# mokemokechicken/reversi-alpha-zero

Hardware: AMD Instinct MI355X
Metric: MCTS simulations/sec (self-play, NN included) (higher is better)
Workload: dtype f64 tree statistics + f32 net (f16x3 split-operand MFMA trunk)

## Files before the change

reversi-alpha-zero_amd/csrc/raz_net_f16x3.hip:

```cpp
#include <hip/hip_runtime.h>
#include <math.h>
#include <stdlib.h>
#include <string.h>
#include <vector>
#include "raz_bitboard.h"
#include "raz_detmath.h"
#include "raz_internal.h"
#include "raz_net_layout.h"

namespace {

typedef _Float16 h8 __attribute__((ext_vector_type(8)));
typedef _Float16 h4 __attribute__((ext_vector_type(4)));
typedef float f32x4 __attribute__((ext_vector_type(4)));
typedef float f32x16 __attribute__((ext_vector_type(16)));

constexpr int OCT = 128;
constexpr int NWAVE = 8;
constexpr int W_STAGE = 3 * 2 * 2 * OCT * 16;
constexpr int ACT_POS = 4 * 64 * 16;
constexpr int ACT_IMG = NWAVE * ACT_POS + 1280;
constexpr int LDS_W = 0;
constexpr int LDS_ACT = 2 * W_STAGE;
constexpr int LDS_BYTES = LDS_ACT + 2 * ACT_IMG;
constexpr int Z_OFF = NWAVE * ACT_POS;

#ifdef RAZ_F16X3_STAMPS
#define RAZ_STAMP_PARAM , unsigned long long* __restrict__ stamps
#define RAZ_STAMP_ARG , (unsigned long long*)nullptr
#define RAZ_STAMP_BEGIN                                                                                           \
    unsigned long long st_t[8];                                                                                   \
    st_t[0] = __builtin_amdgcn_s_memtime();                                                                       \
    st_t[7] = __builtin_amdgcn_s_memrealtime();                                                                   \
    st_t[6] = (unsigned long long)__builtin_amdgcn_s_getreg((4 << 0) | (0 << 6) | (31 << 11)) | ((unsigned long long)__builtin_amdgcn_s_getreg((20 << 0) | (0 << 6) | (31 << 11)) << 32); \
    st_t[5] = 0;                                                                                                  \
    st_t[1] = st_t[2] = st_t[3] = st_t[4] = 0;                                                                    \
    unsigned long long st_b = 0
#define RAZ_STAMP_BARRIER_IN st_b = __builtin_amdgcn_s_memtime()
#define RAZ_STAMP_BARRIER_OUT(st_)                                    \
    do {                                                              \
        const unsigned long long t_ = __builtin_amdgcn_s_memtime();   \
        st_t[5] += t_ - st_b;                                         \
        if ((st_) == 0) st_t[1] = t_;                                 \
    } while (0)
#define RAZ_STAMP_AT(i_) st_t[i_] = __builtin_amdgcn_s_memtime()
#define RAZ_STAMP_END                                                                                    \
    do {                                                                                                 \
        st_t[3] = __builtin_amdgcn_s_memtime();                                                          \
        __builtin_amdgcn_s_waitcnt(0x0070);                                                \
        st_t[4] = __builtin_amdgcn_s_memtime();                                                          \
        if (lane == 0 && stamps)                                                                         \
            for (int i_ = 0; i_ < 8; ++i_) stamps[((size_t)blockIdx.x * NWAVE + wv) * 8 + i_] = st_t[i_]; \
    } while (0)
#else
#define RAZ_STAMP_PARAM
#define RAZ_STAMP_ARG
#define RAZ_STAMP_BEGIN
#define RAZ_STAMP_BARRIER_IN
#define RAZ_STAMP_BARRIER_OUT(st_)
#define RAZ_STAMP_AT(i_)
#define RAZ_STAMP_END
#endif

__device__ __forceinline__ void halves_trade(float a, float b, int upper, float& first, float& second) {
#ifdef RAZ_WAVE_EMU
    const float got = __shfl_xor(upper ? a : b, 32);
    first = upper ? got : a;
    second = upper ? b : got;
#else
    (void)upper;
    const auto r = __builtin_amdgcn_permlane32_swap(__float_as_uint(a), __float_as_uint(b), false, false);
    first = __uint_as_float(r[0]);
    second = __uint_as_float(r[1]);
#endif
}

#define GLDS16(gptr, lptr)                                                                                      \
    __builtin_amdgcn_global_load_lds((const __attribute__((address_space(1))) void*)(gptr),                     \
                                     (__attribute__((address_space(3))) void*)(lptr), 16, 0, 0)

template <bool SPLIT>
__global__ __launch_bounds__(512, 2) void k_conv3x3_f16x3(const unsigned char* __restrict__ Wl, const float* __restrict__ bias,
                                                          const float* __restrict__ inv_scale_ptr, const unsigned char* in, unsigned char* out,
                                                          const unsigned char* skip, const uint8_t* __restrict__ active, int n, int F,
                                                          unsigned* __restrict__ flag, const uint32_t* __restrict__ n_ptr RAZ_STAMP_PARAM) {
    extern __shared__ __attribute__((aligned(16))) unsigned char lds[];
    const int tid = threadIdx.x, lane = tid & 63, wv = tid >> 6;
    RAZ_STAMP_BEGIN;
    if (n_ptr) n = (int)*n_ptr < n ? (int)*n_ptr : n;
    const int noct = F / OCT, nchunks = F / 16;
    const int b = blockIdx.x;
    const int ot = (b >> 3) % noct;
    const int pg = (b / (8 * noct)) * 8 + (b & 7);
    const int p0 = pg * NWAVE, pos = p0 + wv;
    if (p0 >= n) return;
    const bool live = pos < n && (!active || active[pos]);
    const size_t pos_bytes = (size_t)F * 256;
    const unsigned char* in_pos = in + (size_t)(pos < n ? pos : n - 1) * pos_bytes;
    if (tid < 160) {
        const int im = tid / 80, k = tid % 80;
        ((f32x4*)(lds + LDS_ACT + im * ACT_IMG + Z_OFF))[k] = (f32x4){0.f, 0.f, 0.f, 0.f};
    }
    const int kg = lane >> 5;
    uint32_t boff[2][9];
#pragma unroll
    for (int nt = 0; nt < 2; ++nt) {
        const int sq = nt * 32 + (lane & 31), y = sq >> 3, x = sq & 7;
#pragma unroll
        for (int t = 0; t < 9; ++t) {
            const int yy = y + t / 3 - 1, xx = x + t % 3 - 1;
            const bool ok = yy >= 0 && yy < 8 && xx >= 0 && xx < 8;
            const int s2 = sq + (t / 3 - 1) * 8 + (t % 3 - 1);
            boff[nt][t] = ok ? (uint32_t)(wv * ACT_POS + kg * 2048 + s2 * 16) : (uint32_t)(Z_OFF + (s2 & 15) * 16);
        }
    }
    const uint32_t aoff = (uint32_t)(kg * 4096 + (lane & 31) * 16);
    f32x16 acc[4][2];
#pragma unroll
    for (int m = 0; m < 4; ++m)
#pragma unroll
        for (int nt = 0; nt < 2; ++nt)
#pragma unroll
            for (int r = 0; r < 16; ++r) acc[m][nt][r] = 0.f;
    const unsigned char* wsrc = Wl + (size_t)ot * nchunks * 3 * W_STAGE + lane * 16;
    const unsigned char* asrc = in_pos + lane * 16;
    auto issue = [&](int c, int tg) {
        const int st = c * 3 + tg;
        const unsigned char* src = wsrc + (size_t)st * W_STAGE;
        unsigned char* dst = lds + LDS_W + (st & 1) * W_STAGE;
        if constexpr (SPLIT) {
#pragma unroll
            for (int i = 0; i < 3; ++i) GLDS16(src + (wv * 3 + i) * 1024, dst + (wv * 3 + i) * 1024);
        } else {
            const int p0w = (wv >> 1) * 4 + (wv & 1);
            GLDS16(src + p0w * 1024, dst + p0w * 1024);
            if (wv < 4) GLDS16(src + (p0w + 16) * 1024, dst + (p0w + 16) * 1024);
        }
        if (tg == 0) {
            const unsigned char* a = asrc + (size_t)c * ACT_POS;
            unsigned char* ad = lds + LDS_ACT + (c & 1) * ACT_IMG + wv * ACT_POS;
#pragma unroll
            for (int pl = 0; pl < 4; pl += SPLIT ? 1 : 2) GLDS16(a + pl * 1024, ad + pl * 1024);
        }
    };
    issue(0, 0);
    for (int c = 0; c < nchunks; ++c) {
        const uint32_t abase = (uint32_t)(LDS_ACT + (c & 1) * ACT_IMG);
#pragma unroll
        for (int tg = 0; tg < 3; ++tg) {
            const int st = c * 3 + tg;
            RAZ_STAMP_BARRIER_IN;
            __syncthreads();
            RAZ_STAMP_BARRIER_OUT(st);
            if (tg < 2) issue(c, tg + 1);
            else if (c + 1 < nchunks) issue(c + 1, 0);
            const uint32_t wbase = (uint32_t)(LDS_W + (st & 1) * W_STAGE) + aoff;
#pragma unroll
            for (int tt = 0; tt < 3; ++tt) {
                const int t = tg * 3 + tt;
                if constexpr (SPLIT) {
                    h8 bh[2], bl[2];
#pragma unroll
                    for (int nt = 0; nt < 2; ++nt) {
                        bh[nt] = *(const h8*)(lds + abase + boff[nt][t]);
                        bl[nt] = *(const h8*)(lds + abase + boff[nt][t] + 1024);
                    }
#pragma unroll
                    for (int m = 0; m < 4; ++m) {
                        const h8 ah = *(const h8*)(lds + wbase + tt * 8192 + m * 512);
                        const h8 al = *(const h8*)(lds + wbase + tt * 8192 + m * 512 + 2048);
#pragma unroll
                        for (int nt = 0; nt < 2; ++nt) {
                            acc[m][nt] = __builtin_amdgcn_mfma_f32_32x32x16_f16(al, bh[nt], acc[m][nt], 0, 0, 0);
                            acc[m][nt] = __builtin_amdgcn_mfma_f32_32x32x16_f16(ah, bl[nt], acc[m][nt], 0, 0, 0);
                            acc[m][nt] = __builtin_amdgcn_mfma_f32_32x32x16_f16(ah, bh[nt], acc[m][nt], 0, 0, 0);
                        }
                    }
                } else {
                    h8 bh[2];
#pragma unroll
                    for (int nt = 0; nt < 2; ++nt) bh[nt] = *(const h8*)(lds + abase + boff[nt][t]);
#pragma unroll
                    for (int m = 0; m < 4; ++m) {
                        const h8 ah = *(const h8*)(lds + wbase + tt * 8192 + m * 512);
#pragma unroll
                        for (int nt = 0; nt < 2; ++nt) acc[m][nt] = __builtin_amdgcn_mfma_f32_32x32x16_f16(ah, bh[nt], acc[m][nt], 0, 0, 0);
                    }
                }
            }
        }
    }
    RAZ_STAMP_AT(2);
    if (!live) return;
    const float inv_scale = *inv_scale_ptr;
    unsigned char* out_pos = out + (size_t)pos * pos_bytes + lane * 16;
    const unsigned char* skip_pos = skip ? skip + (size_t)pos * pos_bytes + lane * 16 : nullptr;
    h8 skh[2][4], skl[2][4];
    auto load_skip = [&](int m) {
#pragma unroll
        for (int q = 0; q < 4; ++q) {
            const int oc8 = ot * OCT + m * 32 + q * 8;
            const size_t unit = (size_t)(oc8 >> 4) * ACT_POS + (size_t)((oc8 >> 3) & 1) * 2048;
            skh[m & 1][q] = *(const h8*)(skip_pos + unit);
            if constexpr (SPLIT) skl[m & 1][q] = *(const h8*)(skip_pos + unit + 1024);
        }
    };
    if (skip_pos) load_skip(0);
    bool over = false;
#pragma unroll
    for (int m = 0; m < 4; ++m) {
        if (skip_pos && m + 1 < 4) load_skip(m + 1);
#pragma unroll
        for (int q = 0; q < 4; ++q) {
            const int oc8 = ot * OCT + m * 32 + q * 8;
            const size_t unit = (size_t)(oc8 >> 4) * ACT_POS + (size_t)((oc8 >> 3) & 1) * 2048;
            float v[8];
#pragma unroll
            for (int j = 0; j < 4; ++j) halves_trade(acc[m][0][q * 4 + j], acc[m][1][q * 4 + j], kg, v[j], v[4 + j]);
#pragma unroll
            for (int j = 0; j < 8; ++j) v[j] = v[j] * inv_scale + bias[oc8 + j];
            if (skip_pos) {
                const h8 sh = skh[m & 1][q];
                if constexpr (SPLIT) {
                    const h8 sl = skl[m & 1][q];
#pragma unroll
                    for (int j = 0; j < 8; ++j) v[j] = v[j] + ((float)sh[j] + (float)sl[j]);
                } else {
#pragma unroll
                    for (int j = 0; j < 8; ++j) v[j] = v[j] + (float)sh[j];
                }
            }
            h8 hi, lo;
#pragma unroll
            for (int j = 0; j < 8; ++j) {
                const float r = v[j] > 0.0f ? v[j] : 0.0f;
                over |= !(r < 60000.0f);
                hi[j] = (_Float16)r;
                lo[j] = (_Float16)(r - (float)hi[j]);
            }
            *(h8*)(out_pos + unit) = hi;
            if constexpr (SPLIT) *(h8*)(out_pos + unit + 1024) = lo;
        }
    }
    if (over) flag[(size_t)pos * RAZ_NET_ROWFLAG_WORDS] = 1u;
    RAZ_STAMP_END;
}

typedef float f32x2 __attribute__((ext_vector_type(2)));
constexpr int CONV0_ROWS = 2;

template <bool SPLIT>
__global__ __launch_bounds__(256, 6) void k_conv0_split(const float* __restrict__ W0, const raz_bb* __restrict__ own,
                                                        const raz_bb* __restrict__ enemy, const uint8_t* __restrict__ active,
                                                        unsigned char* out, int n, int F, unsigned* __restrict__ flag,
                                                        const uint32_t* __restrict__ list, const uint32_t* __restrict__ n_ptr) {
    const int posA = blockIdx.x * CONV0_ROWS, posB = posA + 1, lane = threadIdx.x & 63;
    const int wv = __builtin_amdgcn_readfirstlane(threadIdx.x >> 6);
    if (threadIdx.x == 0) {
        flag[(size_t)posA * RAZ_NET_ROWFLAG_WORDS] = 0u;
        if (posB < n) flag[(size_t)posB * RAZ_NET_ROWFLAG_WORDS] = 0u;
        if (posA == 0) flag[1] = 0u;
    }
    __syncthreads();
    if (n_ptr) n = (int)*n_ptr < n ? (int)*n_ptr : n;
    const bool liveA = posA < n && (list || !active || active[posA]);
    const bool liveB = posB < n && (list || !active || active[posB]);
    if (!liveA && !liveB) return;
    raz_bb bo[2] = {0, 0}, be[2] = {0, 0};
    if (liveA) {
        const size_t src = list ? list[posA] : (size_t)posA;
        bo[0] = own[src];
        be[0] = enemy[src];
    }
    if (liveB) {
        const size_t src = list ? list[posB] : (size_t)posB;
        bo[1] = own[src];
        be[1] = enemy[src];
    }
    const int y = lane >> 3, x = lane & 7;
    f32x2 x0[9], x1[9];
#pragma unroll
    for (int t = 0; t < 9; ++t) {
        const int yy = y + t / 3 - 1, xx = x + t % 3 - 1;
        const bool ok = (yy >= 0) && (yy < 8) && (xx >= 0) && (xx < 8);
        const int s = (yy * 8 + xx) & 63;
#pragma unroll
        for (int k = 0; k < 2; ++k) {
            x0[t][k] = ok ? (float)(uint32_t)((bo[k] >> s) & 1) : 0.0f;
            x1[t][k] = ok ? (float)(uint32_t)((be[k] >> s) & 1) : 0.0f;
        }
    }
    const float* bias = W0 + (size_t)F * 18;
    unsigned char* op = out + (size_t)posA * F * 256 + lane * 16;
    bool overA = false, overB = false;
    for (int ocb = wv; ocb < F / 16; ocb += 4) {
#pragma unroll 1
        for (int g = 0; g < 2; ++g) {
            f32x2 acc[8];
#pragma unroll
            for (int o = 0; o < 8; ++o) {
                const float b = bias[ocb * 16 + g * 8 + o];
                acc[o] = (f32x2){b, b};
            }
#pragma unroll
            for (int t = 0; t < 9; ++t) {
                const float* wt = W0 + ((size_t)ocb * 9 + t) * 32 + g * 8;
#pragma unroll
                for (int o = 0; o < 8; ++o) {
                    const float w = wt[o];
                    acc[o] = __builtin_elementwise_fma(x0[t], (f32x2){w, w}, acc[o]);
                }
#pragma unroll
                for (int o = 0; o < 8; ++o) {
                    const float w = wt[16 + o];
                    acc[o] = __builtin_elementwise_fma(x1[t], (f32x2){w, w}, acc[o]);
                }
            }
#pragma unroll
            for (int k = 0; k < 2; ++k) {
                if (!(k ? liveB : liveA)) continue;
                h8 hi, lo;
                bool over = false;
#pragma unroll
                for (int j = 0; j < 8; ++j) {
                    const float r = acc[j][k] > 0.0f ? acc[j][k] : 0.0f;
                    over |= !(r < 60000.0f);
                    hi[j] = (_Float16)r;
                    lo[j] = (_Float16)(r - (float)hi[j]);
                }
                if (k) overB |= over;
                else overA |= over;
                unsigned char* o16 = op + (size_t)k * F * 256 + (size_t)ocb * ACT_POS + (g * 2) * 1024;
                *(h8*)o16 = hi;
                if constexpr (SPLIT) *(h8*)(o16 + 1024) = lo;
            }
        }
    }
    if (overA) flag[(size_t)posA * RAZ_NET_ROWFLAG_WORDS] = 1u;
    if (overB) flag[(size_t)posB * RAZ_NET_ROWFLAG_WORDS] = 1u;
}

template <bool SPLIT>
__global__ __launch_bounds__(64) void k_heads_split(const float* __restrict__ H, const unsigned char* trunk,
                                                    const uint8_t* __restrict__ active, float* __restrict__ policy,
                                                    float* __restrict__ value, int n, int F, int V,
                                                    const uint32_t* __restrict__ list, const uint32_t* __restrict__ n_ptr) {
    extern __shared__ __attribute__((aligned(16))) float head[];
    const int pos = blockIdx.x, lane = threadIdx.x;
    if (n_ptr) n = (int)*n_ptr < n ? (int)*n_ptr : n;
    if (pos >= n || (!list && active && !active[pos])) return;
    const size_t dst = list ? list[pos] : (size_t)pos;
    const float* pol_w = H;
    const float* pol_b = pol_w + 2 * F;
    const float* pfc_w = pol_b + 2;
    const float* pfc_b = pfc_w + 128 * 64;
    const float* val_w = pfc_b + 64;
    const float* val_b = val_w + F;
    const float* v1_w = val_b + 1;
    const float* v1_b = v1_w + 64 * V;
    const float* v2_w = v1_b + V;
    const float* v2_b = v2_w + V;
    float* ph = head;
    float* vh = head + 128;
    float* h1 = head + 192;
    const unsigned char* a = trunk + (size_t)pos * F * 256 + lane * 16;
    float p0 = pol_b[0], p1 = pol_b[1], v0 = val_b[0];
    for (int c = 0; c < F / 16; ++c) {
#pragma unroll
        for (int g = 0; g < 2; ++g) {
            const h8 hi = *(const h8*)(a + (size_t)c * ACT_POS + (g * 2 + 0) * 1024);
            h8 lo = hi;
            if constexpr (SPLIT) lo = *(const h8*)(a + (size_t)c * ACT_POS + (g * 2 + 1) * 1024);
#pragma unroll
            for (int j = 0; j < 8; ++j) {
                const int ic = c * 16 + g * 8 + j;
                const float xv = SPLIT ? (float)hi[j] + (float)lo[j] : (float)hi[j];
                p0 = fmaf(xv, pol_w[ic], p0);
                p1 = fmaf(xv, pol_w[F + ic], p1);
                v0 = fmaf(xv, val_w[ic], v0);
            }
        }
    }
    ph[lane] = p0 > 0.0f ? p0 : 0.0f;
    ph[64 + lane] = p1 > 0.0f ? p1 : 0.0f;
    vh[lane] = v0 > 0.0f ? v0 : 0.0f;
    __syncthreads();
    float logit = pfc_b[lane];
#pragma unroll 16
    for (int j = 0; j < 128; ++j) logit = fmaf(ph[j], pfc_w[j * 64 + lane], logit);
    float m = logit;
#pragma unroll
    for (int s = 1; s < 64; s <<= 1) m = fmaxf(m, __shfl_xor(m, s));
    const float e = raz_det_expf(logit - m);
    float sum = e;
#pragma unroll
    for (int s = 1; s < 64; s <<= 1) sum = sum + __shfl_xor(sum, s);
    policy[dst * 64 + lane] = e / sum;
    for (int o0 = 0; o0 < V; o0 += 64) {
        const int o = o0 + lane;
        if (o < V) {
            float acc = v1_b[o];
#pragma unroll 8
            for (int j = 0; j < 64; ++j) acc = fmaf(vh[j], v1_w[j * V + o], acc);
            h1[o] = acc > 0.0f ? acc : 0.0f;
        }
    }
    __syncthreads();
    float acc = v2_b[0];
    for (int j = 0; j < V; ++j) acc = fmaf(h1[j], v2_w[j], acc);
    if (lane == 0) value[dst] = raz_det_tanhf(acc);
}

}

void raz_net_build_f16x3(const float* src, float* dst, int F, int R, int V) {
    const float* lsrc = src + ((size_t)F * 18 + F);
    float* scales = dst + f16x3_scale_off(F, R, V);
    const int nchunks = F / 16, noct = F / 128;
    for (int l = 1; l < 2 * R + 1; ++l) {
        float mx = 0.f;
        for (size_t i = 0; i < (size_t)F * F * 9; ++i) mx = fmaxf(mx, fabsf(lsrc[i]));
        int e = 0;
        if (mx > 0.f) frexpf(mx, &e);
        const float S = ldexpf(1.0f, 15 - e);
        scales[l - 1] = ldexpf(1.0f, e - 15);
        _Float16* w = (_Float16*)(dst + f16x3_layer_off(F, R, V, l));
        for (int ot = 0; ot < noct; ++ot)
            for (int c = 0; c < nchunks; ++c)
                for (int t = 0; t < 9; ++t)
                    for (int kg = 0; kg < 2; ++kg)
                        for (int o = 0; o < 128; ++o)
                            for (int j = 0; j < 8; ++j) {
                                const int oc = ot * 128 + o, ic = c * 16 + kg * 8 + j;
                                const float v = lsrc[((size_t)oc * F + ic) * 9 + t] * S;
                                const _Float16 hi = (_Float16)v, lo = (_Float16)(v - (float)hi);
                                const size_t stage = ((size_t)ot * nchunks + c) * 3 + t / 3;
                                const size_t base = stage * (W_STAGE / 2) + ((size_t)(t % 3) * 2 + kg) * 2 * 128 * 8;
                                w[base + (size_t)o * 8 + j] = hi;
                                w[base + 128 * 8 + (size_t)o * 8 + j] = lo;
                            }
        lsrc += (size_t)F * F * 9 + F;
    }
}

static int heads_launch(bool split, const float* W, int F, int R, int V, const unsigned char* trunk, const uint8_t* active, float* policy,
                        float* value, size_t n, hipStream_t s, const uint32_t* list, const uint32_t* n_ptr) {
    const auto heads = split ? k_heads_split<true> : k_heads_split<false>;
    hipLaunchKernelGGL(heads, dim3((unsigned)n), dim3(64), (192 + (size_t)V) * sizeof(float), s,
                       W + heads_off(F, R), trunk, active, policy, value, (int)n, F, V, list, n_ptr);
    return raz_check_launch("raz_net_forward (split heads)");
}
int raz_net_heads_split(const float* W, int F, int R, int V, const unsigned char* trunk, const uint8_t* active, float* policy, float* value,
                        size_t n, hipStream_t s, const uint32_t* list, const uint32_t* n_ptr) {
    return heads_launch(true, W, F, R, V, trunk, active, policy, value, n, s, list, n_ptr);
}

size_t raz_net_f16x3_scratch_bytes(int F, size_t n) { return n * ((size_t)2 * F * 256 + RAZ_NET_ROWFLAG_WORDS * 4); }

__global__ __launch_bounds__(256) void k_flag_unrepaired(const unsigned* __restrict__ rowflag, unsigned* __restrict__ sticky, int n,
                                                         const uint32_t* __restrict__ n_ptr) {
    const int i = blockIdx.x * 256 + threadIdx.x;
    const int rows = n_ptr ? ((int)*n_ptr < n ? (int)*n_ptr : n) : n;
    if (i < rows && rowflag[(size_t)i * RAZ_NET_ROWFLAG_WORDS]) atomicOr(sticky, 1u);
}
static int raz_net_flag_unrepaired(const unsigned* rowflag, unsigned* sticky, size_t n, const uint32_t* n_ptr, hipStream_t s) {
    hipLaunchKernelGGL(k_flag_unrepaired, dim3((unsigned)((n + 255) / 256)), dim3(256), 0, s, rowflag, sticky, (int)n, n_ptr);
    return raz_check_launch("raz_net_forward (range flags)");
}

unsigned* raz_net_f16x3_flag(const float* W, int F, int R, int V) { return (unsigned*)(W + f16x3_scale_off(F, R, V) + (size_t)2 * R + 8); }

int raz_net_forward_f16x3(const float* W, int F, int R, int V, const uint64_t* own, const uint64_t* enemy,
                          const uint8_t* active, float* policy, float* value, size_t n, void* scratch, size_t scratch_bytes,
                          hipStream_t s, const uint32_t* list, const uint32_t* n_ptr, bool split) {
    if (!scratch || scratch_bytes < raz_net_f16x3_scratch_bytes(F, n))
        return raz_fail(RAZ_ENOMEM, "raz_net_forward: scratch too small (raz_net_scratch_bytes)");
    unsigned char* bufA = (unsigned char*)scratch;
    unsigned char* bufT = bufA + (size_t)n * F * 256;
    unsigned* sticky = raz_net_f16x3_flag(W, F, R, V);
    unsigned* flag = (unsigned*)(bufT + (size_t)n * F * 256);
    const float* scales = W + f16x3_scale_off(F, R, V);
    const auto conv = split ? k_conv3x3_f16x3<true> : k_conv3x3_f16x3<false>;
    {
        static unsigned long long attr_devices[2] = {0, 0};
        int dev = 0;
        RAZ_HIP_TRY(hipGetDevice(&dev), "raz_net_forward: hipGetDevice");
        if (dev >= 64 || !(attr_devices[split] >> dev & 1)) {
            RAZ_HIP_TRY(hipFuncSetAttribute((const void*)conv, hipFuncAttributeMaxDynamicSharedMemorySize, LDS_BYTES), "raz_net_forward: hipFuncSetAttribute");
            if (dev < 64) attr_devices[split] |= 1ull << dev;
        }
    }
    const unsigned conv_threads = NWAVE * 64;
    const auto conv0 = split ? k_conv0_split<true> : k_conv0_split<false>;
    hipLaunchKernelGGL(conv0, dim3((unsigned)((n + CONV0_ROWS - 1) / CONV0_ROWS)), dim3(256), 0, s, W + conv_off(F, 0), (const raz_bb*)own,
                       (const raz_bb*)enemy, active, bufA, (int)n, F, flag, list, n_ptr);
    const unsigned groups = (unsigned)((n + NWAVE - 1) / NWAVE);
    const unsigned tiles = ((groups + 7) / 8) * 8 * (unsigned)(F / 128);
    const unsigned grid = tiles;
    for (int r = 0; r < R; ++r) {
        const int l1 = 1 + 2 * r, l2 = 2 + 2 * r;
        hipLaunchKernelGGL(conv, dim3(grid), dim3(conv_threads), LDS_BYTES, s,
                           (const unsigned char*)(W + f16x3_layer_off(F, R, V, l1)), W + conv_off(F, l1) + (size_t)F * 9 * F,
                           scales + (l1 - 1), (const unsigned char*)bufA, bufT, (const unsigned char*)nullptr, list ? nullptr : active, (int)n, F, flag, n_ptr RAZ_STAMP_ARG);
        hipLaunchKernelGGL(conv, dim3(grid), dim3(conv_threads), LDS_BYTES, s,
                           (const unsigned char*)(W + f16x3_layer_off(F, R, V, l2)), W + conv_off(F, l2) + (size_t)F * 9 * F,
                           scales + (l2 - 1), (const unsigned char*)bufT, bufA, (const unsigned char*)bufA, list ? nullptr : active, (int)n, F, flag, n_ptr RAZ_STAMP_ARG);
    }
    const int rc = heads_launch(split, W, F, R, V, bufA, active, policy, value, n, s, list, n_ptr);
    if (rc != RAZ_OK) return rc;
    if (!f16x3_repairs(F, V))
        return raz_net_flag_unrepaired(flag, sticky, n, n_ptr, s);
    return raz_net_repair_rows(W, F, R, V, own, enemy, policy, value, n, flag, sticky, list, n_ptr, s);
}
```

Measured before the change: 375,500.

## Remap conv3x3 waves to row-strip tiles across positions with padded LDS layout

Restructures the 3x3 conv MFMA tiling. Previously each wave handled one position over all 128 output channels. Now each wave covers 64 output channels, half the board rows, and columns drawn from 4 positions, reusing activation rows across vertical taps via compile-time row-shifted stages. The per-position LDS activation images are padded by 128 bytes and the zero region is enlarged, presumably to reduce bank conflicts and register-held offsets (boff shrinks from 18 entries to 3). The epilogue is remapped so each lane writes its own position, with liveness checked per lane. This adds branchy stage dispatch and a more complex output mapping.

```diff
diff --git a/reversi-alpha-zero_amd/csrc/raz_net_f16x3.hip b/reversi-alpha-zero_amd/csrc/raz_net_f16x3.hip
--- a/reversi-alpha-zero_amd/csrc/raz_net_f16x3.hip
+++ b/reversi-alpha-zero_amd/csrc/raz_net_f16x3.hip
@@ -19,11 +19,13 @@
 constexpr int NWAVE = 8;
 constexpr int W_STAGE = 3 * 2 * 2 * OCT * 16;
 constexpr int ACT_POS = 4 * 64 * 16;
-constexpr int ACT_IMG = NWAVE * ACT_POS + 1280;
+constexpr int Z_OFF = NWAVE * (ACT_POS + 128);
+constexpr int Z_BYTES = 2048;
+constexpr int ACT_IMG = Z_OFF + Z_BYTES;
 constexpr int LDS_W = 0;
 constexpr int LDS_ACT = 2 * W_STAGE;
 constexpr int LDS_BYTES = LDS_ACT + 2 * ACT_IMG;
-constexpr int Z_OFF = NWAVE * ACT_POS;
+constexpr int act_pos_off(int p) { return p * (ACT_POS + 128); }
 
 #ifdef RAZ_F16X3_STAMPS
 #define RAZ_STAMP_PARAM , unsigned long long* __restrict__ stamps
@@ -79,13 +81,45 @@
     __builtin_amdgcn_global_load_lds((const __attribute__((address_space(1))) void*)(gptr),                     \
                                      (__attribute__((address_space(3))) void*)(lptr), 16, 0, 0)
 
+template <bool SPLIT, int TG, int J0, int J1>
+__device__ __forceinline__ void conv_stage(const unsigned char* lds, uint32_t wbase, uint32_t abase, const uint32_t (&boff)[3],
+                                           f32x16 (&acc)[2][4]) {
+#pragma unroll
+    for (int tt = 0; tt < 3; ++tt) {
+        h8 bh[4], bl[4];
+#pragma unroll
+        for (int j = J0; j < J1; ++j) {
+            const uint32_t at = abase + boff[tt] + (j + TG) * 128;
+            bh[j] = *(const h8*)(lds + at);
+            if constexpr (SPLIT) bl[j] = *(const h8*)(lds + at + 1024);
+        }
+#pragma unroll
+        for (int m = 0; m < 2; ++m) {
+            const h8 ah = *(const h8*)(lds + wbase + tt * 8192 + m * 512);
+            if constexpr (SPLIT) {
+                const h8 al = *(const h8*)(lds + wbase + tt * 8192 + m * 512 + 2048);
+#pragma unroll
+                for (int j = J0; j < J1; ++j) {
+                    acc[m][j] = __builtin_amdgcn_mfma_f32_32x32x16_f16(al, bh[j], acc[m][j], 0, 0, 0);
+                    acc[m][j] = __builtin_amdgcn_mfma_f32_32x32x16_f16(ah, bl[j], acc[m][j], 0, 0, 0);
+                    acc[m][j] = __builtin_amdgcn_mfma_f32_32x32x16_f16(ah, bh[j], acc[m][j], 0, 0, 0);
+                }
+            } else {
+#pragma unroll
+                for (int j = J0; j < J1; ++j) acc[m][j] = __builtin_amdgcn_mfma_f32_32x32x16_f16(ah, bh[j], acc[m][j], 0, 0, 0);
+            }
+        }
+    }
+}
+
 template <bool SPLIT>
 __global__ __launch_bounds__(512, 2) void k_conv3x3_f16x3(const unsigned char* __restrict__ Wl, const float* __restrict__ bias,
                                                           const float* __restrict__ inv_scale_ptr, const unsigned char* in, unsigned char* out,
                                                           const unsigned char* skip, const uint8_t* __restrict__ active, int n, int F,
                                                           unsigned* __restrict__ flag, const uint32_t* __restrict__ n_ptr RAZ_STAMP_PARAM) {
     extern __shared__ __attribute__((aligned(16))) unsigned char lds[];
-    const int tid = threadIdx.x, lane = tid & 63, wv = tid >> 6;
+    const int tid = threadIdx.x, lane = tid & 63;
+    const int wv = __builtin_amdgcn_readfirstlane(tid >> 6);
     RAZ_STAMP_BEGIN;
     if (n_ptr) n = (int)*n_ptr < n ? (int)*n_ptr : n;
     const int noct = F / OCT, nchunks = F / 16;
@@ -94,34 +128,29 @@
     const int pg = (b / (8 * noct)) * 8 + (b & 7);
     const int p0 = pg * NWAVE, pos = p0 + wv;
     if (p0 >= n) return;
-    const bool live = pos < n && (!active || active[pos]);
     const size_t pos_bytes = (size_t)F * 256;
     const unsigned char* in_pos = in + (size_t)(pos < n ? pos : n - 1) * pos_bytes;
-    if (tid < 160) {
-        const int im = tid / 80, k = tid % 80;
+    if (tid < 2 * (Z_BYTES / 16)) {
+        const int im = tid / (Z_BYTES / 16), k = tid % (Z_BYTES / 16);
         ((f32x4*)(lds + LDS_ACT + im * ACT_IMG + Z_OFF))[k] = (f32x4){0.f, 0.f, 0.f, 0.f};
     }
-    const int kg = lane >> 5;
-    uint32_t boff[2][9];
-#pragma unroll
-    for (int nt = 0; nt < 2; ++nt) {
-        const int sq = nt * 32 + (lane & 31), y = sq >> 3, x = sq & 7;
-#pragma unroll
-        for (int t = 0; t < 9; ++t) {
-            const int yy = y + t / 3 - 1, xx = x + t % 3 - 1;
-            const bool ok = yy >= 0 && yy < 8 && xx >= 0 && xx < 8;
-            const int s2 = sq + (t / 3 - 1) * 8 + (t % 3 - 1);
-            boff[nt][t] = ok ? (uint32_t)(wv * ACT_POS + kg * 2048 + s2 * 16) : (uint32_t)(Z_OFF + (s2 & 15) * 16);
-        }
-    }
-    const uint32_t aoff = (uint32_t)(kg * 4096 + (lane & 31) * 16);
-    f32x16 acc[4][2];
-#pragma unroll
-    for (int m = 0; m < 4; ++m)
-#pragma unroll
-        for (int nt = 0; nt < 2; ++nt)
-#pragma unroll
-            for (int r = 0; r < 16; ++r) acc[m][nt][r] = 0.f;
+    const int half = wv >> 2, grp = (wv >> 1) & 1, oh = wv & 1;
+    const int kg = lane >> 5, colpos = grp * 4 + ((lane & 31) >> 3), x = lane & 7;
+    uint32_t boff[3];
+#pragma unroll
+    for (int t = 0; t < 3; ++t) {
+        const int xx = x + t - 1;
+        const int at = act_pos_off(colpos) + kg * 2048 + ((4 * half - 1) * 8 + xx) * 16;
+        boff[t] = xx >= 0 && xx < 8 ? (uint32_t)at : (uint32_t)(Z_OFF + (at & 255));
+    }
+    const uint32_t aoff = (uint32_t)(kg * 4096 + oh * 1024 + (lane & 31) * 16);
+    f32x16 acc[2][4];
+#pragma unroll
+    for (int m = 0; m < 2; ++m)
+#pragma unroll
+        for (int j = 0; j < 4; ++j)
+#pragma unroll
+            for (int r = 0; r < 16; ++r) acc[m][j][r] = 0.f;
     const unsigned char* wsrc = Wl + (size_t)ot * nchunks * 3 * W_STAGE + lane * 16;
     const unsigned char* asrc = in_pos + lane * 16;
     auto issue = [&](int c, int tg) {
@@ -138,7 +167,7 @@
         }
         if (tg == 0) {
             const unsigned char* a = asrc + (size_t)c * ACT_POS;
-            unsigned char* ad = lds + LDS_ACT + (c & 1) * ACT_IMG + wv * ACT_POS;
+            unsigned char* ad = lds + LDS_ACT + (c & 1) * ACT_IMG + act_pos_off(wv);
 #pragma unroll
             for (int pl = 0; pl < 4; pl += SPLIT ? 1 : 2) GLDS16(a + pl * 1024, ad + pl * 1024);
         }
@@ -155,74 +184,55 @@
             if (tg < 2) issue(c, tg + 1);
             else if (c + 1 < nchunks) issue(c + 1, 0);
             const uint32_t wbase = (uint32_t)(LDS_W + (st & 1) * W_STAGE) + aoff;
-#pragma unroll
-            for (int tt = 0; tt < 3; ++tt) {
-                const int t = tg * 3 + tt;
-                if constexpr (SPLIT) {
-                    h8 bh[2], bl[2];
-#pragma unroll
-                    for (int nt = 0; nt < 2; ++nt) {
-                        bh[nt] = *(const h8*)(lds + abase + boff[nt][t]);
-                        bl[nt] = *(const h8*)(lds + abase + boff[nt][t] + 1024);
-                    }
-#pragma unroll
-                    for (int m = 0; m < 4; ++m) {
-                        const h8 ah = *(const h8*)(lds + wbase + tt * 8192 + m * 512);
-                        const h8 al = *(const h8*)(lds + wbase + tt * 8192 + m * 512 + 2048);
-#pragma unroll
-                        for (int nt = 0; nt < 2; ++nt) {
-                            acc[m][nt] = __builtin_amdgcn_mfma_f32_32x32x16_f16(al, bh[nt], acc[m][nt], 0, 0, 0);
-                            acc[m][nt] = __builtin_amdgcn_mfma_f32_32x32x16_f16(ah, bl[nt], acc[m][nt], 0, 0, 0);
-                            acc[m][nt] = __builtin_amdgcn_mfma_f32_32x32x16_f16(ah, bh[nt], acc[m][nt], 0, 0, 0);
-                        }
-                    }
-                } else {
-                    h8 bh[2];
-#pragma unroll
-                    for (int nt = 0; nt < 2; ++nt) bh[nt] = *(const h8*)(lds + abase + boff[nt][t]);
-#pragma unroll
-                    for (int m = 0; m < 4; ++m) {
-                        const h8 ah = *(const h8*)(lds + wbase + tt * 8192 + m * 512);
-#pragma unroll
-                        for (int nt = 0; nt < 2; ++nt) acc[m][nt] = __builtin_amdgcn_mfma_f32_32x32x16_f16(ah, bh[nt], acc[m][nt], 0, 0, 0);
-                    }
-                }
+            if (tg == 0) {
+                conv_stage<SPLIT, 0, 1, 4>(lds, wbase, abase, boff, acc);
+                if (half != 0) conv_stage<SPLIT, 0, 0, 1>(lds, wbase, abase, boff, acc);
+            } else if (tg == 1) {
+                conv_stage<SPLIT, 1, 0, 4>(lds, wbase, abase, boff, acc);
+            } else {
+                conv_stage<SPLIT, 2, 0, 3>(lds, wbase, abase, boff, acc);
+                if (half != 1) conv_stage<SPLIT, 2, 3, 4>(lds, wbase, abase, boff, acc);
             }
         }
     }
     RAZ_STAMP_AT(2);
-    if (!live) return;
+    const int lpos = p0 + colpos;
+    const bool live = lpos < n && (!active || active[lpos]);
+    if (!__any(live)) return;
     const float inv_scale = *inv_scale_ptr;
-    unsigned char* out_pos = out + (size_t)pos * pos_bytes + lane * 16;
-    const unsigned char* skip_pos = skip ? skip + (size_t)pos * pos_bytes + lane * 16 : nullptr;
+    const size_t lane_off = (size_t)(live ? lpos : p0) * pos_bytes + (size_t)((4 * half + kg) * 8 + x) * 16;
+    unsigned char* out_pos = out + lane_off;
+    const unsigned char* skip_pos = skip ? skip + lane_off : nullptr;
     h8 skh[2][4], skl[2][4];
-    auto load_skip = [&](int m) {
+    auto load_skip = [&](int it) {
 #pragma unroll
         for (int q = 0; q < 4; ++q) {
-            const int oc8 = ot * OCT + m * 32 + q * 8;
-            const size_t unit = (size_t)(oc8 >> 4) * ACT_POS + (size_t)((oc8 >> 3) & 1) * 2048;
-            skh[m & 1][q] = *(const h8*)(skip_pos + unit);
-            if constexpr (SPLIT) skl[m & 1][q] = *(const h8*)(skip_pos + unit + 1024);
+            const int oc8 = ot * OCT + oh * 64 + (it >> 1) * 32 + q * 8;
+            const size_t unit = (size_t)(oc8 >> 4) * ACT_POS + (size_t)((oc8 >> 3) & 1) * 2048 + (size_t)(it & 1) * 256;
+            skh[it & 1][q] = *(const h8*)(skip_pos + unit);
+            if constexpr (SPLIT) skl[it & 1][q] = *(const h8*)(skip_pos + unit + 1024);
         }
     };
-    if (skip_pos) load_skip(0);
+    if (skip_pos && live) load_skip(0);
     bool over = false;
 #pragma unroll
-    for (int m = 0; m < 4; ++m) {
-        if (skip_pos && m + 1 < 4) load_skip(m + 1);
+    for (int it = 0; it < 4; ++it) {
+        const int m = it >> 1, k = it & 1;
+        if (skip_pos && live && it + 1 < 4) load_skip(it + 1);
 #pragma unroll
         for (int q = 0; q < 4; ++q) {
-            const int oc8 = ot * OCT + m * 32 + q * 8;
-            const size_t unit = (size_t)(oc8 >> 4) * ACT_POS + (size_t)((oc8 >> 3) & 1) * 2048;
+            const int oc8 = ot * OCT + oh * 64 + m * 32 + q * 8;
+            const size_t unit = (size_t)(oc8 >> 4) * ACT_POS + (size_t)((oc8 >> 3) & 1) * 2048 + (size_t)k * 256;
             float v[8];
 #pragma unroll
-            for (int j = 0; j < 4; ++j) halves_trade(acc[m][0][q * 4 + j], acc[m][1][q * 4 + j], kg, v[j], v[4 + j]);
+            for (int j = 0; j < 4; ++j) halves_trade(acc[m][2 * k][q * 4 + j], acc[m][2 * k + 1][q * 4 + j], kg, v[j], v[4 + j]);
+            if (!live) continue;
 #pragma unroll
             for (int j = 0; j < 8; ++j) v[j] = v[j] * inv_scale + bias[oc8 + j];
             if (skip_pos) {
-                const h8 sh = skh[m & 1][q];
+                const h8 sh = skh[it & 1][q];
                 if constexpr (SPLIT) {
-                    const h8 sl = skl[m & 1][q];
+                    const h8 sl = skl[it & 1][q];
 #pragma unroll
                     for (int j = 0; j < 8; ++j) v[j] = v[j] + ((float)sh[j] + (float)sl[j]);
                 } else {
@@ -242,7 +252,7 @@
             if constexpr (SPLIT) *(h8*)(out_pos + unit + 1024) = lo;
         }
     }
-    if (over) flag[(size_t)pos * RAZ_NET_ROWFLAG_WORDS] = 1u;
+    if (live && over) flag[(size_t)lpos * RAZ_NET_ROWFLAG_WORDS] = 1u;
     RAZ_STAMP_END;
 }
 
```

New measurement: 397,600, median of 6. 1.06x the previous value.
